# hyeeiin/ECG-Multimodal-Model

Hardware: AMD Instinct MI355X
Metric: samples/sec fwd+bwd, batch-256 multimodal (img+sig+clin), 1->8 MI355X (higher is better)
Workload: dtype bf16; 1 GPU; full multimodal (image 3x224x224 + 5000-pt signal + 16-dim clinical), fwd+bwd+Adam, encoders unfrozen; image_hw=224x224, per_gpu_batch=256, global_batch=256, parallelism=dp1

## Files before the change

ecg-multimodal-model_amd/csrc/conv_stem.hip:

```cpp
#include "ops.h"

__device__ __host__ inline size_t align_up_dev(size_t a) { return (a + 15) & ~(size_t)15; }

#ifndef STEM_ABL
#define STEM_ABL 0
#endif

namespace {

constexpr int STEM_CO = 64;
constexpr int MAXG = 24;

struct StemParams {
  const float* x;
  const void* wpk;
  void* y;
  const float* bias;
  float* stats;
  float* slab;
  int N, Cin, H, W, OH, OW, R, pad_h;
  int TH, TW;
  int tiles_h, tiles_w;
  int NG;
};

template <typename T> struct StemCfg;
template <> struct StemCfg<bf16_t> { static constexpr int WPAD = 8; };
template <> struct StemCfg<float> { static constexpr int WPAD = 4; };

template <int R> struct StemDims {
  static constexpr int TH = R == 1 ? 1 : 8, TW = R == 1 ? 128 : 16;
  static constexpr int PH = (TH - 1) * 2 + R, PW = (TW - 1) * 2 + 8, PWS = (PW + 1) & ~1;
  static constexpr int NPRE = R == 1 ? 16 : 10;
};

template <int R>
__device__ __forceinline__ void stem_patch_offsets(const StemParams& p, int oh0, int ow0,
                                                   unsigned (&off)[StemDims<R>::NPRE]) {
  constexpr int PH = StemDims<R>::PH, PW = StemDims<R>::PW, PWS = StemDims<R>::PWS, NPRE = StemDims<R>::NPRE;
  const int total = p.Cin * PH * PWS;
  const int ih0 = oh0 * 2 - p.pad_h, iw0 = ow0 * 2 - 3;
#pragma unroll
  for (int k = 0; k < NPRE; ++k) {
    const int i = threadIdx.x + 256 * k;
    const int pw = i % PWS;
    const int t = i / PWS;
    const int ph = t % PH, c = t / PH;
    const int ih = ih0 + ph, iw = iw0 + pw;
    const int ok = (int)(i < total) & (int)(pw < PW) & (int)((unsigned)ih < (unsigned)p.H) &
                   (int)((unsigned)iw < (unsigned)p.W);
    off[k] = ok ? (unsigned)((c * p.H + ih) * p.W + iw) * 4u : 0xFFFFFFFFu;
  }
}
template <int R>
__device__ __forceinline__ void stem_fetch_image_patch(const StemParams& p, const unsigned (&off)[StemDims<R>::NPRE],
                                                       float (&pre)[StemDims<R>::NPRE], int n) {
  const size_t img = (size_t)p.Cin * p.H * p.W;
  const __amdgpu_buffer_rsrc_t rs = __builtin_amdgcn_make_buffer_rsrc((void*)(p.x + (size_t)n * img), 0,
                                                                      (int)(img * sizeof(float)), 0x00020000);
#pragma unroll
  for (int k = 0; k < StemDims<R>::NPRE; ++k) {
#if defined(__HIP_DEVICE_COMPILE__)
    pre[k] = __builtin_bit_cast(float, __builtin_amdgcn_raw_buffer_load_b32(rs, (int)off[k], 0, 0));
#endif
  }
}
template <typename T, int R>
__device__ __forceinline__ void stem_store_slots(T* patch, const float (&pre)[StemDims<R>::NPRE]) {
#pragma unroll
  for (int k = 0; k < StemDims<R>::NPRE; ++k) {
    if constexpr (sizeof(T) == 2) patch[threadIdx.x + 256 * k] = f2bf(pre[k]);
    else patch[threadIdx.x + 256 * k] = pre[k];
  }
}

__device__ __forceinline__ int stem_xcd_order() {
  const int nwg = gridDim.x, q = nwg >> 3, r = nwg & 7, xcd = blockIdx.x & 7, k = blockIdx.x >> 3;
  return (xcd < r ? xcd * (q + 1) : r * (q + 1) + (xcd - r) * q) + k;
}

template <typename T, int R, int SMODE = 0>
__global__ __launch_bounds__(256) void stem_fwd_kernel(StemParams p) {
  constexpr bool STATS_ONLY = SMODE == 1, STATS_WG = SMODE != 0;
  extern __shared__ __attribute__((aligned(16))) unsigned char smem[];
  constexpr int TH = StemDims<R>::TH, TW = StemDims<R>::TW, PH = StemDims<R>::PH, PWS = StemDims<R>::PWS;
  constexpr int NPRE = StemDims<R>::NPRE, PB = NPRE * 256;
  constexpr int VEC = Elem<T>::VEC;
  constexpr int KSMAX = (MAXG + 3) / 4;
  const int ksteps = (p.NG + 3) / 4;
  const int KP = ksteps * 32;
  const int WS = KP + StemCfg<T>::WPAD;
  T* sW = reinterpret_cast<T*>(smem);
  T* const patch0 = reinterpret_cast<T*>(smem + align_up_dev((size_t)STEM_CO * WS * sizeof(T)));

  const int tid = threadIdx.x, lane = tid & 63, wave = tid >> 6;
  const int fr = lane & 15, fq = lane >> 4;

  {
    const T* wg = (const T*)p.wpk;
    const int vpr = KP / VEC;
    for (int i = tid; i < STEM_CO * vpr; i += 256) {
      int co = i / vpr, kv = i - co * vpr;
      *reinterpret_cast<u32x4*>(sW + co * WS + kv * VEC) = *reinterpret_cast<const u32x4*>(wg + (size_t)co * KP + kv * VEC);
    }
  }
  const int tpi = p.tiles_h * p.tiles_w;
  const int vb = stem_xcd_order();
  const int pos = vb % tpi, slot = vb / tpi, nslots = gridDim.x / tpi;
  const int th_i = pos / p.tiles_w, tw_i = pos - th_i * p.tiles_w;
  const int oh0 = th_i * TH, ow0 = tw_i * TW;

  float pre[NPRE];
  unsigned poff[NPRE];
  stem_patch_offsets<R>(p, oh0, ow0, poff);

  constexpr int segs = TW / 16;
  int prow[2], pcol[2], boff[2], oofs[2];
  bool okb[2];
#pragma unroll
  for (int b = 0; b < 2; ++b) {
    const int t = wave * 2 + b;
    prow[b] = t / segs;
    pcol[b] = (t % segs) * 16 + fr;
    boff[b] = prow[b] * 2 * PWS + pcol[b] * 2;
    okb[b] = (oh0 + prow[b] < p.OH) & (ow0 + pcol[b] < p.OW);
    oofs[b] = ((oh0 + prow[b]) * p.OW + ow0 + pcol[b]) * STEM_CO;
  }
  unsigned goff2[KSMAX / 2];
#pragma unroll
  for (int ks = 0; ks < KSMAX; ++ks) {
    int G = ks * 4 + fq;
    if (G >= p.NG) G = p.NG - 1;
    const int c = G / R, r = G - c * R;
    const unsigned g = (unsigned)((c * PH + r) * PWS);
    if (ks & 1) goff2[ks / 2] |= g << 16;
    else goff2[ks / 2] = g;
  }
  const T* wlane = sW + fr * WS + fq * 8;

  float ws1[STATS_WG ? 4 : 1][4], ws2[STATS_WG ? 4 : 1][4];
  if (STATS_WG) {
#pragma unroll
    for (int a = 0; a < 4; ++a)
#pragma unroll
      for (int j = 0; j < 4; ++j) ws1[a][j] = ws2[a][j] = 0.f;
  }
  int n = slot;
  if (n < p.N) {
    stem_fetch_image_patch<R>(p, poff, pre, n);
    stem_store_slots<T, R>(patch0, pre);
  }
  __syncthreads();
  for (int cur = 0; n < p.N; n += nslots, cur ^= 1) {
  const T* patch = patch0 + cur * PB;
  const bool has_next = n + nslots < p.N;
  if (has_next && (STEM_ABL != 4 || p.N < 0)) stem_fetch_image_patch<R>(p, poff, pre, n + nslots);

  f32x4 acc[4][2];
  if constexpr (sizeof(T) != 2) {
#pragma unroll
    for (int a = 0; a < 4; ++a)
#pragma unroll
      for (int b = 0; b < 2; ++b) acc[a][b] = (f32x4){0.f, 0.f, 0.f, 0.f};
  }

  if constexpr (sizeof(T) == 2) {
#pragma unroll
    for (int ks = 0; ks < KSMAX; ++ks) {
      if (ks < ksteps && (STEM_ABL != 3 || p.N < 0)) {
        u32x4 fb[2];
#pragma unroll
        for (int b = 0; b < 2; ++b) {
          const int goff = (ks & 1) ? (int)(goff2[ks / 2] >> 16) : (int)(goff2[ks / 2] & 0xffffu);
          const unsigned* src = reinterpret_cast<const unsigned*>(patch + goff + boff[b]);
          fb[b] = (u32x4){src[0], src[1], src[2], src[3]};
        }
#pragma unroll
        for (int a = 0; a < 4; ++a) {
          u32x4 fa = *reinterpret_cast<const u32x4*>(wlane + a * 16 * WS + ks * 32);
#pragma unroll
          for (int b = 0; b < 2; ++b) {
            if (ks == 0) mfma_bf16_first(acc[a][b], fa, fb[b]);
            else mfma_bf16_inplace(acc[a][b], fa, fb[b]);
          }
        }
      }
    }
    mfma_drain();
  } else {
    for (int ks = 0; ks < ksteps; ++ks) {
#pragma unroll
      for (int g = 0; g < 4; ++g) {
        int G2 = ks * 4 + g;
        if (G2 >= p.NG) G2 = p.NG - 1;
        const int c2 = G2 / R, r2 = G2 - c2 * R;
#pragma unroll
        for (int hf = 0; hf < 2; ++hf) {
          const int s = hf * 4 + fq;
          float fbv[2];
#pragma unroll
          for (int b = 0; b < 2; ++b) fbv[b] = patch[(c2 * PH + r2) * PWS + boff[b] + s];
#pragma unroll
          for (int a = 0; a < 4; ++a) {
            float fav = sW[(a * 16 + fr) * WS + (ks * 4 + g) * 8 + s];
#pragma unroll
            for (int b = 0; b < 2; ++b)
              acc[a][b] = __builtin_amdgcn_mfma_f32_16x16x4f32(fav, fbv[b], acc[a][b], 0, 0, 0);
          }
        }
      }
    }
  }

  if (has_next) stem_store_slots<T, R>(patch0 + (cur ^ 1) * PB, pre);
  if constexpr (STATS_ONLY) {
#pragma unroll
    for (int a = 0; a < 4; ++a)
#pragma unroll
      for (int b = 0; b < 2; ++b)
        if (okb[b]) {
#pragma unroll
          for (int j = 0; j < 4; ++j) {
            const float v = p.bias ? acc[a][b][j] + p.bias[a * 16 + fq * 4 + j] : acc[a][b][j];
            ws1[a][j] += v;
            ws2[a][j] += v * v;
          }
        }
    __syncthreads();
    continue;
  }
  T* yimg = (T*)p.y + (size_t)n * p.OH * p.OW * STEM_CO;
  const int tile = n * tpi + pos;
  const __amdgpu_buffer_rsrc_t yrs = __builtin_amdgcn_make_buffer_rsrc(
      (void*)yimg, 0, (int)((size_t)p.OH * p.OW * STEM_CO * sizeof(T)), 0x00020000);
  const __amdgpu_buffer_rsrc_t srs = __builtin_amdgcn_make_buffer_rsrc(
      (void*)(p.stats ? p.stats + (size_t)tile * 4 * 2 * STEM_CO : nullptr), 0, p.stats ? 4 * 2 * STEM_CO * 4 : 0, 0x00020000);
#pragma unroll
  for (int ap = 0; ap < 4; ap += 2) {
  uint2 opk[2][2];
#pragma unroll
  for (int a = ap; a < ap + 2; ++a) {
    const int ch0 = a * 16 + fq * 4;
    float bvv[4] = {0.f, 0.f, 0.f, 0.f};
    if (p.bias) {
#pragma unroll
      for (int j = 0; j < 4; ++j) bvv[j] = p.bias[ch0 + j];
    }
    float s1[4] = {0.f, 0.f, 0.f, 0.f}, s2[4] = {0.f, 0.f, 0.f, 0.f};
#pragma unroll
    for (int b = 0; b < 2; ++b) {
      float v[4];
#pragma unroll
      for (int j = 0; j < 4; ++j) v[j] = p.bias ? acc[a][b][j] + bvv[j] : acc[a][b][j];
      if (okb[b]) {
#pragma unroll
        for (int j = 0; j < 4; ++j) {
          s1[j] += v[j];
          s2[j] += v[j] * v[j];
        }
        if (sizeof(T) != 2) *reinterpret_cast<float4*>(yimg + oofs[b] + ch0) = make_float4(v[0], v[1], v[2], v[3]);
      }
      if (sizeof(T) == 2) {
        opk[a - ap][b].x = (unsigned)f2bf(v[0]) | ((unsigned)f2bf(v[1]) << 16);
        opk[a - ap][b].y = (unsigned)f2bf(v[2]) | ((unsigned)f2bf(v[3]) << 16);
      }
    }
    if (STATS_WG) {
      if (p.stats) {
#pragma unroll
        for (int j = 0; j < 4; ++j) {
          ws1[a][j] += s1[j];
          ws2[a][j] += s2[j];
        }
      }
    } else if (p.stats && (STEM_ABL != 2 || p.N < 0)) {
#pragma unroll
      for (int j = 0; j < 4; ++j) {
        s1[j] = row16_sum(s1[j]);
        s2[j] = row16_sum(s2[j]);
      }
#if defined(__HIP_DEVICE_COMPILE__)
      {
        const unsigned so = fr == 0 ? (unsigned)((wave * 2 * STEM_CO + ch0) * 4) : 0xFFFFFFFFu;
        __builtin_amdgcn_raw_buffer_store_b128((u32x4){__float_as_uint(s1[0]), __float_as_uint(s1[1]), __float_as_uint(s1[2]), __float_as_uint(s1[3])},
                                               srs, (int)so, 0, 0);
        __builtin_amdgcn_raw_buffer_store_b128((u32x4){__float_as_uint(s2[0]), __float_as_uint(s2[1]), __float_as_uint(s2[2]), __float_as_uint(s2[3])},
                                               srs, (int)so, STEM_CO * 4, 0);
      }
#endif
    }
  }
#if defined(__HIP_DEVICE_COMPILE__)
  if (sizeof(T) == 2) {
#pragma unroll
    for (int b = 0; b < 2; ++b) {
      auto lo = __builtin_amdgcn_permlane16_swap(opk[0][b].x, opk[1][b].x, false, false);
      auto hi = __builtin_amdgcn_permlane16_swap(opk[0][b].y, opk[1][b].y, false, false);
      const int ch = (fq & 1) ? (ap + 1) * 16 + (fq - 1) * 4 : ap * 16 + fq * 4;
      const unsigned yo = okb[b] ? (unsigned)(oofs[b] + ch) * 2u : 0xFFFFFFFFu;
      if (STEM_ABL != 1 || p.N < 0)
        __builtin_amdgcn_raw_buffer_store_b128((u32x4){lo[0], hi[0], lo[1], hi[1]}, yrs, (int)yo, 0, 0);
    }
  }
#endif
  }
  __syncthreads();
  }
  if (STATS_WG && p.stats) {
    float* srow = p.stats + ((size_t)blockIdx.x * 4 + wave) * 2 * STEM_CO;
#pragma unroll
    for (int a = 0; a < 4; ++a) {
      f32x4 r1, r2;
#pragma unroll
      for (int j = 0; j < 4; ++j) {
        r1[j] = row16_sum(ws1[a][j]);
        r2[j] = row16_sum(ws2[a][j]);
      }
      if (fr == 0) {
        *reinterpret_cast<f32x4*>(srow + a * 16 + fq * 4) = r1;
        *reinterpret_cast<f32x4*>(srow + STEM_CO + a * 16 + fq * 4) = r2;
      }
    }
  }
}

template <typename T, int R>
__global__ __launch_bounds__(256) void stem_wgrad_kernel(StemParams p) {
  extern __shared__ __attribute__((aligned(16))) unsigned char smem[];
  constexpr int DYS = sizeof(T) == 2 ? 144 : 320;
  constexpr int TH = StemDims<R>::TH, TW = StemDims<R>::TW, PH = StemDims<R>::PH, PWS = StemDims<R>::PWS;
  unsigned char* sDY = smem;
  float* patch = reinterpret_cast<float*>(smem + 128 * DYS);

  const int tid = threadIdx.x, lane = tid & 63, wave = tid >> 6;
  const int fr = lane & 15, fq = lane >> 4;
  const int NK = p.NG * 8;
  const int ktiles = (NK + 15) / 16;
  const int tpi = p.tiles_h * p.tiles_w;
  const int vb = stem_xcd_order();
  const int pos = vb % tpi, slot = vb / tpi, nslots = gridDim.x / tpi;
  const int th_i = pos / p.tiles_w, tw_i = pos - th_i * p.tiles_w;
  const int oh0 = th_i * TH, ow0 = tw_i * TW;

  f32x4 acc[4][3];
#pragma unroll
  for (int a = 0; a < 4; ++a)
#pragma unroll
    for (int b = 0; b < 3; ++b) acc[a][b] = (f32x4){0.f, 0.f, 0.f, 0.f};

  int koff[3];
#pragma unroll
  for (int b = 0; b < 3; ++b) {
    const int kidx = (wave + 4 * b) * 16 + fr;
    const bool kok = (wave + 4 * b) < ktiles && kidx < NK;
    const int kk = kok ? kidx : 0;
    const int G = kk >> 3, c = G / R;
    koff[b] = (c * PH + (G - c * R)) * PWS + (kk & 7);
  }

  const T* dy = (const T*)p.y;
  constexpr int CH = 64 * (int)sizeof(T) / 16;
  constexpr int NDY = 128 * CH / 256;
  float pre[StemDims<R>::NPRE];
  u32x4 pdy[NDY];
  unsigned poff[StemDims<R>::NPRE], dyoff[NDY];
  stem_patch_offsets<R>(p, oh0, ow0, poff);
#pragma unroll
  for (int k = 0; k < NDY; ++k) {
    const int i = tid + 256 * k;
    const int pix = i / CH, chunk = i % CH;
    const int oh = oh0 + pix / TW, ow = ow0 + pix % TW;
    dyoff[k] = ((oh < p.OH) & (ow < p.OW)) ? (unsigned)(((oh * p.OW + ow) * STEM_CO) * (int)sizeof(T) + chunk * 16) : 0xFFFFFFFFu;
  }
  auto fetch = [&](int n) {
    const size_t dimg = (size_t)p.OH * p.OW * STEM_CO;
    const __amdgpu_buffer_rsrc_t drs = __builtin_amdgcn_make_buffer_rsrc((void*)(dy + (size_t)n * dimg), 0,
                                                                          (int)(dimg * sizeof(T)), 0x00020000);
#pragma unroll
    for (int k = 0; k < NDY; ++k) {
#if defined(__HIP_DEVICE_COMPILE__)
      pdy[k] = __builtin_amdgcn_raw_buffer_load_b128(drs, (int)dyoff[k], 0, 0);
#endif
    }
    stem_fetch_image_patch<R>(p, poff, pre, n);
  };
  if (slot < p.N) fetch(slot);
  for (int n = slot; n < p.N; n += nslots) {
    __syncthreads();
#pragma unroll
    for (int k = 0; k < NDY; ++k) {
      const int i = tid + 256 * k;
      *reinterpret_cast<u32x4*>(sDY + (i / CH) * DYS + (i % CH) * 16) = pdy[k];
    }
    stem_store_slots<float, R>(patch, pre);
    __syncthreads();
    if (n + nslots < p.N) fetch(n + nslots);

    if constexpr (sizeof(T) == 2) {
      const int q = fr >> 2, pq = fr & 3;
      for (int st = 0; st < 4; ++st) {
        u32x4 fa[4];
#pragma unroll
        for (int a = 0; a < 4; ++a) {
          const unsigned char* a0 = sDY + (st * 32 + 8 * fq + q) * DYS + (a * 16 + 4 * pq) * 2;
          s16x4 lo = __builtin_amdgcn_ds_read_tr16_b64_v4i16(
              (__attribute__((address_space(3))) s16x4*)(const_cast<unsigned char*>(a0)));
          s16x4 hi = __builtin_amdgcn_ds_read_tr16_b64_v4i16(
              (__attribute__((address_space(3))) s16x4*)(const_cast<unsigned char*>(a0 + 4 * DYS)));
          uint2 l2 = __builtin_bit_cast(uint2, lo), h2 = __builtin_bit_cast(uint2, hi);
          fa[a] = (u32x4){l2.x, l2.y, h2.x, h2.y};
        }
        const int pix0 = st * 32 + 8 * fq;
        const int trow = pix0 / TW, tcol0 = pix0 % TW;
#pragma unroll
        for (int b = 0; b < 3; ++b) {
          float bv[8];
          const float* src = patch + koff[b] + trow * 2 * PWS + tcol0 * 2;
#pragma unroll
          for (int j = 0; j < 8; ++j) bv[j] = src[2 * j];
          u32x4 fb = pack16<bf16_t>(bv);
#pragma unroll
          for (int a = 0; a < 4; ++a)
            mfma_bf16_inplace(acc[a][b], fa[a], fb);
        }
      }
    } else {
      for (int st = 0; st < 32; ++st) {
        const int pix = st * 4 + fq;
        const int trow = pix / TW, tcol = pix % TW;
        float fa[4];
#pragma unroll
        for (int a = 0; a < 4; ++a) fa[a] = *reinterpret_cast<const float*>(sDY + pix * DYS + (a * 16 + fr) * 4);
#pragma unroll
        for (int b = 0; b < 3; ++b) {
          float fb = patch[koff[b] + trow * 2 * PWS + tcol * 2];
#pragma unroll
          for (int a = 0; a < 4; ++a) acc[a][b] = __builtin_amdgcn_mfma_f32_16x16x4f32(fa[a], fb, acc[a][b], 0, 0, 0);
        }
      }
    }
  }

  if (sizeof(T) == 2) mfma_drain();
#pragma unroll
  for (int b = 0; b < 3; ++b) {
    int kidx = (wave + 4 * b) * 16 + fr;
    if ((wave + 4 * b) >= ktiles || kidx >= NK) continue;
#pragma unroll
    for (int a = 0; a < 4; ++a)
#pragma unroll
      for (int j = 0; j < 4; ++j)
        p.slab[((size_t)blockIdx.x * STEM_CO + a * 16 + fq * 4 + j) * NK + kidx] = acc[a][b][j];
  }
}

__global__ __launch_bounds__(256) void stem_wgrad_reduce_kernel(const float* __restrict__ slab,
                                                                float* __restrict__ grad, int nsplit, int NG,
                                                                int accumulate) {
  __shared__ float sh[16][17];
  const int oi = threadIdx.x & 15, sl = threadIdx.x >> 4;
  const int i = blockIdx.x * 16 + oi;
  const int total = STEM_CO * NG * 7;
  const int NK = NG * 8;
  float acc = 0.f;
  if (i < total) {
    int s = i % 7;
    int t = i / 7;
    int G = t % NG, co = t / NG;
    const float* src = slab + (size_t)co * NK + G * 8 + s;
    const size_t stride = (size_t)STEM_CO * NK;
    int k = sl;
    for (; k + 48 < nsplit; k += 64) {
      const float a0 = src[(size_t)k * stride], a1 = src[(size_t)(k + 16) * stride];
      const float a2 = src[(size_t)(k + 32) * stride], a3 = src[(size_t)(k + 48) * stride];
      acc += a0;
      acc += a1;
      acc += a2;
      acc += a3;
    }
    for (; k < nsplit; k += 16) acc += src[(size_t)k * stride];
  }
  sh[sl][oi] = acc;
  __syncthreads();
  if (sl == 0 && i < total) {
    float v = 0.f;
    for (int k = 0; k < 16; ++k) v += sh[k][oi];
    grad[i] = accumulate ? grad[i] + v : v;
  }
}

template <typename T>
__global__ void stem_pack_kernel(const float* __restrict__ w, T* __restrict__ out, int NG, int KP) {
  int i = blockIdx.x * blockDim.x + threadIdx.x;
  if (i >= STEM_CO * KP) return;
  int co = i / KP, k = i - co * KP;
  int G = k >> 3, s = k & 7;
  float v = (G < NG && s < 7) ? w[((size_t)co * NG + G) * 7 + s] : 0.f;
  Elem<T>::st(out + i, v);
}

struct StemShape {
  int OH, OW, TH, TW, tiles_h, tiles_w, NG, KP;
};
int stem_shape(int Cin, int H, int W, int R, StemShape& s) {
  if (R != 1 && R != 7) ECG_FAIL(ECGMM_ERR_SHAPE, "stem: R=%d (1 or 7)", R);
  s.NG = Cin * R;
  if (s.NG > MAXG) ECG_FAIL(ECGMM_ERR_SHAPE, "stem: Cin*R=%d > %d", s.NG, MAXG);
  int pad_h = R / 2;
  s.OH = (H + 2 * pad_h - R) / 2 + 1;
  s.OW = (W + 6 - 7) / 2 + 1;
  if (R == 1) { s.TH = 1; s.TW = 128; }
  else { s.TH = 8; s.TW = 16; }
  s.tiles_h = ceil_div(s.OH, s.TH);
  s.tiles_w = ceil_div(s.OW, s.TW);
  s.KP = ((s.NG + 3) / 4) * 32;
  {
    int PH = (s.TH - 1) * 2 + R, PW = (s.TW - 1) * 2 + 8, PWS = (PW + 1) & ~1;
    if ((double)Cin * H * W * 4.0 >= 2147483648.0 || (double)s.OH * s.OW * STEM_CO * 4.0 >= 2147483648.0)
      ECG_FAIL(ECGMM_ERR_SHAPE, "stem: one sample of %d x %d x %d exceeds the 2 GiB buffer-addressing range", Cin, H, W);
    if (Cin * PH * PWS > (R == 1 ? 16 : 10) * 256) ECG_FAIL(ECGMM_ERR_SHAPE, "stem: input patch of %d channels exceeds the prefetch registers", Cin);
  }
  return 0;
}
void fill_params(StemParams& p, const StemShape& s, int N, int Cin, int H, int W, int R) {
  memset(&p, 0, sizeof(p));
  p.N = N; p.Cin = Cin; p.H = H; p.W = W; p.OH = s.OH; p.OW = s.OW; p.R = R; p.pad_h = R / 2;
  p.TH = s.TH; p.TW = s.TW; p.tiles_h = s.tiles_h; p.tiles_w = s.tiles_w; p.NG = s.NG;
}
size_t stem_patch_buffer_bytes(int R, size_t esz) { return (size_t)(R == 1 ? 16 : 10) * 256 * esz; }
size_t patch_bytes(const StemShape& s, int Cin, int R) {
  int PH = (s.TH - 1) * 2 + R, PW = (s.TW - 1) * 2 + 8, PWS = (PW + 1) & ~1;
  return (size_t)Cin * PH * PWS * sizeof(float);
}

}

size_t ecg_stem_packed_elems(int Cin, int R) { return (size_t)STEM_CO * (((Cin * R + 3) / 4) * 32); }
int ecg_stem_stats_rows(int N, int Cin, int H, int W, int R) {
  StemShape s;
  if (stem_shape(Cin, H, W, R, s)) return -1;
  return 4 * N * s.tiles_h * s.tiles_w;
}

int ecg_stem_pack(int dtype, const float* w, void* out, int Cin, int R, hipStream_t stream) {
  int NG = Cin * R, KP = ((NG + 3) / 4) * 32;
  int n = STEM_CO * KP;
  if (dtype == ECGMM_BF16)
    hipLaunchKernelGGL(stem_pack_kernel<bf16_t>, dim3(ceil_div(n, 256)), dim3(256), 0, stream, w, (bf16_t*)out, NG, KP);
  else
    hipLaunchKernelGGL(stem_pack_kernel<float>, dim3(ceil_div(n, 256)), dim3(256), 0, stream, w, (float*)out, NG, KP);
  ECG_CHECK_LAUNCH("stem_pack");
  return 0;
}

int ecg_stem_wg_stats_rows(int N, int Cin, int H, int W, int R) { return ecg_stem_stats_only_rows(N, Cin, H, W, R); }
static int stem_fwd_impl(int dtype, const float* x, const void* wpk, const float* bias, void* y, float* stats, int N, int Cin,
                         int H, int W, int R, bool wg_rows, hipStream_t stream);
int ecg_stem_fwd_wgrows(int dtype, const float* x, const void* wpk, const float* bias, void* y, float* stats, int N, int Cin,
                        int H, int W, int R, hipStream_t stream) {
  return stem_fwd_impl(dtype, x, wpk, bias, y, stats, N, Cin, H, W, R, true, stream);
}
int ecg_stem_fwd(int dtype, const float* x, const void* wpk, const float* bias, void* y, float* stats, int N, int Cin,
                 int H, int W, int R, hipStream_t stream) {
  return stem_fwd_impl(dtype, x, wpk, bias, y, stats, N, Cin, H, W, R, false, stream);
}
static int stem_fwd_impl(int dtype, const float* x, const void* wpk, const float* bias, void* y, float* stats, int N, int Cin,
                         int H, int W, int R, bool wg_rows, hipStream_t stream) {
  StemShape s;
  ECG_TRY(stem_shape(Cin, H, W, R, s));
  StemParams p;
  fill_params(p, s, N, Cin, H, W, R);
  p.x = x; p.wpk = wpk; p.y = y; p.bias = bias; p.stats = stats;
  const size_t esz = dtype_size(dtype);
  const int WS = s.KP + (dtype == ECGMM_BF16 ? 8 : 4);
  size_t lds = align_up((size_t)STEM_CO * WS * esz, 16) + 2 * stem_patch_buffer_bytes(R, esz);
  const int tpi = s.tiles_h * s.tiles_w;
  int nslots = 2048 / tpi;
  nslots = nslots < 1 ? 1 : (nslots > N ? N : nslots);
  dim3 grid(tpi * nslots);
  ecg_prof_begin(ECG_PROF_STEM_FWD, 2.0 * (double)N * s.OH * s.OW * STEM_CO * Cin * R * 7,
                 4.0 * N * Cin * H * W + (double)dtype_size(dtype) * N * s.OH * s.OW * STEM_CO, stream);
  if (dtype == ECGMM_BF16 && wg_rows) {
    if (R == 7) hipLaunchKernelGGL((stem_fwd_kernel<bf16_t, 7, 2>), grid, dim3(256), lds, stream, p);
    else hipLaunchKernelGGL((stem_fwd_kernel<bf16_t, 1, 2>), grid, dim3(256), lds, stream, p);
  } else if (wg_rows) {
    ECG_FAIL(ECGMM_ERR_DTYPE, "stem: per-workgroup statistics rows are a bf16 form");
  } else if (dtype == ECGMM_BF16) {
    if (R == 7) hipLaunchKernelGGL((stem_fwd_kernel<bf16_t, 7>), grid, dim3(256), lds, stream, p);
    else hipLaunchKernelGGL((stem_fwd_kernel<bf16_t, 1>), grid, dim3(256), lds, stream, p);
  } else if (dtype == ECGMM_F32) {
    static bool once = false;
    if (!once) {
      (void)hipFuncSetAttribute((const void*)stem_fwd_kernel<float, 7>, hipFuncAttributeMaxDynamicSharedMemorySize, 100 * 1024);
      (void)hipFuncSetAttribute((const void*)stem_fwd_kernel<float, 1>, hipFuncAttributeMaxDynamicSharedMemorySize, 100 * 1024);
      once = true;
    }
    if (R == 7) hipLaunchKernelGGL((stem_fwd_kernel<float, 7>), grid, dim3(256), lds, stream, p);
    else hipLaunchKernelGGL((stem_fwd_kernel<float, 1>), grid, dim3(256), lds, stream, p);
  } else {
    ECG_FAIL(ECGMM_ERR_DTYPE, "stem: bad dtype %d", dtype);
  }
  ecg_prof_end(stream);
  ECG_CHECK_LAUNCH("stem_fwd");
  return 0;
}

static int stem_stats_grid(int N, int tpi) {
  int nslots = 2048 / tpi;
  nslots = nslots < 1 ? 1 : (nslots > N ? N : nslots);
  return tpi * nslots;
}
int ecg_stem_stats_only_rows(int N, int Cin, int H, int W, int R) {
  StemShape s;
  if (stem_shape(Cin, H, W, R, s)) return -1;
  return 4 * stem_stats_grid(N, s.tiles_h * s.tiles_w);
}
int ecg_stem_stats_only(int dtype, const float* x, const void* wpk, const float* bias, float* stats, int N, int Cin,
                        int H, int W, int R, hipStream_t stream) {
  if (dtype != ECGMM_BF16) ECG_FAIL(ECGMM_ERR_DTYPE, "stem statistics-only pass: bf16 only");
  StemShape s;
  ECG_TRY(stem_shape(Cin, H, W, R, s));
  StemParams p;
  fill_params(p, s, N, Cin, H, W, R);
  p.x = x; p.wpk = wpk; p.bias = bias; p.stats = stats;
  const int WS = s.KP + 8;
  size_t lds = align_up((size_t)STEM_CO * WS * 2, 16) + 2 * stem_patch_buffer_bytes(R, 2);
  dim3 grid(stem_stats_grid(N, s.tiles_h * s.tiles_w));
  ecg_prof_begin(ECG_PROF_STEM_FWD, 2.0 * (double)N * s.OH * s.OW * STEM_CO * Cin * R * 7, 4.0 * N * Cin * H * W, stream);
  if (R == 7) hipLaunchKernelGGL((stem_fwd_kernel<bf16_t, 7, 1>), grid, dim3(256), lds, stream, p);
  else hipLaunchKernelGGL((stem_fwd_kernel<bf16_t, 1, 1>), grid, dim3(256), lds, stream, p);
  ecg_prof_end(stream);
  ECG_CHECK_LAUNCH("stem_stats_only");
  return 0;
}

int ecg_stem_wgrad_reduce(const float* slab, float* grad, int rows, int NG, int accumulate, hipStream_t stream) {
  hipLaunchKernelGGL(stem_wgrad_reduce_kernel, dim3(ceil_div(STEM_CO * NG * 7, 16)), dim3(256), 0, stream, slab, grad, rows, NG,
                     accumulate);
  ECG_CHECK_LAUNCH("stem_wgrad_reduce");
  return 0;
}

static int stem_wgrad_grid(int N, int tpi) {
  int nslots = 1024 / tpi;
  nslots = nslots < 1 ? 1 : (nslots > N ? N : nslots);
  return tpi * nslots;
}

size_t ecg_stem_wgrad_workspace(int N, int Cin, int H, int W, int R) {
  StemShape s;
  if (stem_shape(Cin, H, W, R, s)) return 0;
  return (size_t)stem_wgrad_grid(N, s.tiles_h * s.tiles_w) * STEM_CO * s.NG * 8 * sizeof(float);
}

int ecg_stem_wgrad(int dtype, const float* x, const void* dy, float* grad, int accumulate, void* workspace,
                   size_t workspace_bytes, int N, int Cin, int H, int W, int R, hipStream_t stream) {
  StemShape s;
  ECG_TRY(stem_shape(Cin, H, W, R, s));
  const int grid = stem_wgrad_grid(N, s.tiles_h * s.tiles_w);
  size_t need = (size_t)grid * STEM_CO * s.NG * 8 * sizeof(float);
  if (!workspace || workspace_bytes < need)
    ECG_FAIL(ECGMM_ERR_WORKSPACE, "stem wgrad: workspace %zu < %zu", workspace_bytes, need);
  StemParams p;
  fill_params(p, s, N, Cin, H, W, R);
  p.x = x; p.y = const_cast<void*>(dy); p.slab = (float*)workspace;
  size_t lds = 128 * (size_t)(dtype == ECGMM_BF16 ? 144 : 320) + stem_patch_buffer_bytes(R, sizeof(float));
  if (dtype != ECGMM_BF16 && dtype != ECGMM_F32) ECG_FAIL(ECGMM_ERR_DTYPE, "stem wgrad: bad dtype %d", dtype);
  ecg_prof_begin(ECG_PROF_STEM_WGRAD, 2.0 * (double)N * s.OH * s.OW * STEM_CO * Cin * R * 7,
                 4.0 * N * Cin * H * W + (double)dtype_size(dtype) * N * s.OH * s.OW * STEM_CO, stream);
  if (dtype == ECGMM_BF16) {
    if (R == 7) hipLaunchKernelGGL((stem_wgrad_kernel<bf16_t, 7>), dim3(grid), dim3(256), lds, stream, p);
    else hipLaunchKernelGGL((stem_wgrad_kernel<bf16_t, 1>), dim3(grid), dim3(256), lds, stream, p);
  } else {
    if (R == 7) hipLaunchKernelGGL((stem_wgrad_kernel<float, 7>), dim3(grid), dim3(256), lds, stream, p);
    else hipLaunchKernelGGL((stem_wgrad_kernel<float, 1>), dim3(grid), dim3(256), lds, stream, p);
  }
  ecg_prof_end(stream);
  ECG_CHECK_LAUNCH("stem_wgrad");
  hipLaunchKernelGGL(stem_wgrad_reduce_kernel, dim3(ceil_div(STEM_CO * s.NG * 7, 16)), dim3(256), 0, stream,
                     (const float*)workspace, grad, grid, s.NG, accumulate);
  ECG_CHECK_LAUNCH("stem_wgrad_reduce");
  return 0;
}
```

Baseline: 39150 samples/s.

## Specialize stem conv k-steps, cache bias in LDS, parity-split bf16 wgrad patch

```diff
diff --git a/ecg-multimodal-model_amd/csrc/conv_stem.hip b/ecg-multimodal-model_amd/csrc/conv_stem.hip
--- a/ecg-multimodal-model_amd/csrc/conv_stem.hip
+++ b/ecg-multimodal-model_amd/csrc/conv_stem.hip
@@ -32,6 +32,7 @@
   static constexpr int TH = R == 1 ? 1 : 8, TW = R == 1 ? 128 : 16;
   static constexpr int PH = (TH - 1) * 2 + R, PW = (TW - 1) * 2 + 8, PWS = (PW + 1) & ~1;
   static constexpr int NPRE = R == 1 ? 16 : 10;
+  static constexpr int PWH = (PW / 2 + 7) & ~7;
 };
 
 template <int R>
@@ -74,20 +75,41 @@
   }
 }
 
+template <int R>
+__device__ __forceinline__ void stem_parity_slots(const StemParams& p, unsigned (&dst2)[StemDims<R>::NPRE / 2]) {
+  constexpr int PH = StemDims<R>::PH, PWS = StemDims<R>::PWS, PWH = StemDims<R>::PWH, NPRE = StemDims<R>::NPRE;
+  const int total = p.Cin * PH * PWS;
+#pragma unroll
+  for (int k = 0; k < NPRE; ++k) {
+    const int i = threadIdx.x + 256 * k;
+    const int pw = i % PWS, row = i / PWS;
+    const unsigned d = i < total ? (unsigned)((row * 2 + (pw & 1)) * PWH + (pw >> 1)) : (unsigned)(PWH - 1);
+    if (k & 1) dst2[k / 2] |= d << 16;
+    else dst2[k / 2] = d;
+  }
+}
+template <int R>
+__device__ __forceinline__ void stem_store_parity(bf16_t* patch, const float (&pre)[StemDims<R>::NPRE],
+                                                  const unsigned (&dst2)[StemDims<R>::NPRE / 2]) {
+#pragma unroll
+  for (int k = 0; k < StemDims<R>::NPRE; ++k)
+    patch[(k & 1) ? dst2[k / 2] >> 16 : dst2[k / 2] & 0xffffu] = f2bf(pre[k]);
+}
+
 __device__ __forceinline__ int stem_xcd_order() {
   const int nwg = gridDim.x, q = nwg >> 3, r = nwg & 7, xcd = blockIdx.x & 7, k = blockIdx.x >> 3;
   return (xcd < r ? xcd * (q + 1) : r * (q + 1) + (xcd - r) * q) + k;
 }
 
-template <typename T, int R, int SMODE = 0>
+template <typename T, int R, int SMODE = 0, int KS = 0>
 __global__ __launch_bounds__(256) void stem_fwd_kernel(StemParams p) {
   constexpr bool STATS_ONLY = SMODE == 1, STATS_WG = SMODE != 0;
   extern __shared__ __attribute__((aligned(16))) unsigned char smem[];
   constexpr int TH = StemDims<R>::TH, TW = StemDims<R>::TW, PH = StemDims<R>::PH, PWS = StemDims<R>::PWS;
   constexpr int NPRE = StemDims<R>::NPRE, PB = NPRE * 256;
   constexpr int VEC = Elem<T>::VEC;
-  constexpr int KSMAX = (MAXG + 3) / 4;
-  const int ksteps = (p.NG + 3) / 4;
+  constexpr int KSMAX = KS ? KS : (MAXG + 3) / 4;
+  const int ksteps = KS ? KS : (p.NG + 3) / 4;
   const int KP = ksteps * 32;
   const int WS = KP + StemCfg<T>::WPAD;
   T* sW = reinterpret_cast<T*>(smem);
@@ -104,6 +126,8 @@
       *reinterpret_cast<u32x4*>(sW + co * WS + kv * VEC) = *reinterpret_cast<const u32x4*>(wg + (size_t)co * KP + kv * VEC);
     }
   }
+  float* const sBias = reinterpret_cast<float*>(patch0 + 2 * PB);
+  if (p.bias && tid < STEM_CO) sBias[tid] = p.bias[tid];
   const int tpi = p.tiles_h * p.tiles_w;
   const int vb = stem_xcd_order();
   const int pos = vb % tpi, slot = vb / tpi, nslots = gridDim.x / tpi;
@@ -126,7 +150,7 @@
     okb[b] = (oh0 + prow[b] < p.OH) & (ow0 + pcol[b] < p.OW);
     oofs[b] = ((oh0 + prow[b]) * p.OW + ow0 + pcol[b]) * STEM_CO;
   }
-  unsigned goff2[KSMAX / 2];
+  unsigned goff2[(KSMAX + 1) / 2];
 #pragma unroll
   for (int ks = 0; ks < KSMAX; ++ks) {
     int G = ks * 4 + fq;
@@ -164,7 +188,34 @@
       for (int b = 0; b < 2; ++b) acc[a][b] = (f32x4){0.f, 0.f, 0.f, 0.f};
   }
 
-  if constexpr (sizeof(T) == 2) {
+  if constexpr (sizeof(T) == 2 && KS > 0) {
+    if (STEM_ABL != 3 || p.N < 0) {
+      u32x4 fa[2][4], fb[2][2];
+      auto read_step = [&](int ks, u32x4 (&a4)[4], u32x4 (&b2)[2]) {
+        const int goff = (ks & 1) ? (int)(goff2[ks / 2] >> 16) : (int)(goff2[ks / 2] & 0xffffu);
+#pragma unroll
+        for (int b = 0; b < 2; ++b) {
+          const unsigned* src = reinterpret_cast<const unsigned*>(patch + goff + boff[b]);
+          b2[b] = (u32x4){src[0], src[1], src[2], src[3]};
+        }
+#pragma unroll
+        for (int a = 0; a < 4; ++a) a4[a] = *reinterpret_cast<const u32x4*>(wlane + a * 16 * WS + ks * 32);
+      };
+      read_step(0, fa[0], fb[0]);
+#pragma unroll
+      for (int ks = 0; ks < KS; ++ks) {
+        if (ks + 1 < KS) read_step(ks + 1, fa[(ks + 1) & 1], fb[(ks + 1) & 1]);
+#pragma unroll
+        for (int a = 0; a < 4; ++a)
+#pragma unroll
+          for (int b = 0; b < 2; ++b) {
+            if (ks == 0) mfma_bf16_first(acc[a][b], fa[0][a], fb[0][b]);
+            else mfma_bf16_inplace(acc[a][b], fa[ks & 1][a], fb[ks & 1][b]);
+          }
+      }
+    }
+    mfma_drain();
+  } else if constexpr (sizeof(T) == 2) {
 #pragma unroll
     for (int ks = 0; ks < KSMAX; ++ks) {
       if (ks < ksteps && (STEM_ABL != 3 || p.N < 0)) {
@@ -221,7 +272,7 @@
         if (okb[b]) {
 #pragma unroll
           for (int j = 0; j < 4; ++j) {
-            const float v = p.bias ? acc[a][b][j] + p.bias[a * 16 + fq * 4 + j] : acc[a][b][j];
+            const float v = p.bias ? acc[a][b][j] + sBias[a * 16 + fq * 4 + j] : acc[a][b][j];
             ws1[a][j] += v;
             ws2[a][j] += v * v;
           }
@@ -244,7 +295,7 @@
     float bvv[4] = {0.f, 0.f, 0.f, 0.f};
     if (p.bias) {
 #pragma unroll
-      for (int j = 0; j < 4; ++j) bvv[j] = p.bias[ch0 + j];
+      for (int j = 0; j < 4; ++j) bvv[j] = sBias[ch0 + j];
     }
     float s1[4] = {0.f, 0.f, 0.f, 0.f}, s2[4] = {0.f, 0.f, 0.f, 0.f};
 #pragma unroll
@@ -329,8 +380,10 @@
   extern __shared__ __attribute__((aligned(16))) unsigned char smem[];
   constexpr int DYS = sizeof(T) == 2 ? 144 : 320;
   constexpr int TH = StemDims<R>::TH, TW = StemDims<R>::TW, PH = StemDims<R>::PH, PWS = StemDims<R>::PWS;
+  constexpr int PWH = StemDims<R>::PWH;
+  constexpr bool PAR = sizeof(T) == 2;
   unsigned char* sDY = smem;
-  float* patch = reinterpret_cast<float*>(smem + 128 * DYS);
+  T* patch = reinterpret_cast<T*>(smem + 128 * DYS);
 
   const int tid = threadIdx.x, lane = tid & 63, wave = tid >> 6;
   const int fr = lane & 15, fq = lane >> 4;
@@ -355,8 +408,10 @@
     const bool kok = (wave + 4 * b) < ktiles && kidx < NK;
     const int kk = kok ? kidx : 0;
     const int G = kk >> 3, c = G / R;
-    koff[b] = (c * PH + (G - c * R)) * PWS + (kk & 7);
-  }
+    koff[b] = PAR ? ((c * PH + (G - c * R)) * 2 + (kk & 1)) * PWH : (c * PH + (G - c * R)) * PWS + (kk & 7);
+  }
+  const bool sh_dword = (fr & 4) != 0;
+  const unsigned sh_bits = (fr & 2) ? 16u : 0u;
 
   const T* dy = (const T*)p.y;
   constexpr int CH = 64 * (int)sizeof(T) / 16;
@@ -365,6 +420,8 @@
   u32x4 pdy[NDY];
   unsigned poff[StemDims<R>::NPRE], dyoff[NDY];
   stem_patch_offsets<R>(p, oh0, ow0, poff);
+  unsigned pdst2[StemDims<R>::NPRE / 2];
+  if constexpr (PAR) stem_parity_slots<R>(p, pdst2);
 #pragma unroll
   for (int k = 0; k < NDY; ++k) {
     const int i = tid + 256 * k;
@@ -392,14 +449,20 @@
       const int i = tid + 256 * k;
       *reinterpret_cast<u32x4*>(sDY + (i / CH) * DYS + (i % CH) * 16) = pdy[k];
     }
-    stem_store_slots<float, R>(patch, pre);
+    if constexpr (PAR) stem_store_parity<R>(patch, pre, pdst2);
+    else stem_store_slots<float, R>(patch, pre);
     __syncthreads();
     if (n + nslots < p.N) fetch(n + nslots);
 
     if constexpr (sizeof(T) == 2) {
       const int q = fr >> 2, pq = fr & 3;
-      for (int st = 0; st < 4; ++st) {
-        u32x4 fa[4];
+      struct BRaw { u32x4 lo; uint2 hi; };
+      u32x4 fa[4];
+      BRaw fbr[3];
+      const bf16_t* bsrc[3];
+#pragma unroll
+      for (int b = 0; b < 3; ++b) bsrc[b] = patch + koff[b] + (8 * fq / TW) * 4 * PWH + (8 * fq) % TW;
+      auto read_step = [&](int st, u32x4 (&a4)[4], BRaw (&b3)[3]) {
 #pragma unroll
         for (int a = 0; a < 4; ++a) {
           const unsigned char* a0 = sDY + (st * 32 + 8 * fq + q) * DYS + (a * 16 + 4 * pq) * 2;
@@ -408,20 +471,32 @@
           s16x4 hi = __builtin_amdgcn_ds_read_tr16_b64_v4i16(
               (__attribute__((address_space(3))) s16x4*)(const_cast<unsigned char*>(a0 + 4 * DYS)));
           uint2 l2 = __builtin_bit_cast(uint2, lo), h2 = __builtin_bit_cast(uint2, hi);
-          fa[a] = (u32x4){l2.x, l2.y, h2.x, h2.y};
-        }
-        const int pix0 = st * 32 + 8 * fq;
-        const int trow = pix0 / TW, tcol0 = pix0 % TW;
+          a4[a] = (u32x4){l2.x, l2.y, h2.x, h2.y};
+        }
+        static_assert(TW == 16 || TW == 128, "a 32-pixel step is two whole tile rows or a quarter of one");
+        constexpr int STEP = TW == 16 ? 2 * 4 * PWH : 32;
 #pragma unroll
         for (int b = 0; b < 3; ++b) {
-          float bv[8];
-          const float* src = patch + koff[b] + trow * 2 * PWS + tcol0 * 2;
-#pragma unroll
-          for (int j = 0; j < 8; ++j) bv[j] = src[2 * j];
-          u32x4 fb = pack16<bf16_t>(bv);
-#pragma unroll
-          for (int a = 0; a < 4; ++a)
-            mfma_bf16_inplace(acc[a][b], fa[a], fb);
+          const bf16_t* src = bsrc[b] + st * STEP;
+          b3[b].lo = *reinterpret_cast<const u32x4*>(src);
+          b3[b].hi = *reinterpret_cast<const uint2*>(src + 8);
+        }
+      };
+      auto b_frag = [&](const BRaw& r) {
+        auto pick = [&](unsigned d0, unsigned d1) { return sh_dword ? d1 : d0; };
+        const unsigned e0 = pick(r.lo[0], r.lo[1]), e1 = pick(r.lo[1], r.lo[2]), e2 = pick(r.lo[2], r.lo[3]);
+        const unsigned e3 = pick(r.lo[3], r.hi.x), e4 = pick(r.hi.x, r.hi.y);
+        return (u32x4){__builtin_amdgcn_alignbit(e1, e0, sh_bits), __builtin_amdgcn_alignbit(e2, e1, sh_bits),
+                       __builtin_amdgcn_alignbit(e3, e2, sh_bits), __builtin_amdgcn_alignbit(e4, e3, sh_bits)};
+      };
+#pragma unroll
+      for (int st = 0; st < 4; ++st) {
+        read_step(st, fa, fbr);
+#pragma unroll
+        for (int b = 0; b < 3; ++b) {
+          const u32x4 fb = b_frag(fbr[b]);
+#pragma unroll
+          for (int a = 0; a < 4; ++a) mfma_bf16_inplace(acc[a][b], fa[a], fb);
         }
       }
     } else {
@@ -528,6 +603,18 @@
   p.TH = s.TH; p.TW = s.TW; p.tiles_h = s.tiles_h; p.tiles_w = s.tiles_w; p.NG = s.NG;
 }
 size_t stem_patch_buffer_bytes(int R, size_t esz) { return (size_t)(R == 1 ? 16 : 10) * 256 * esz; }
+
+template <int SMODE>
+void stem_fwd_launch_bf16(const StemParams& p, dim3 grid, size_t lds, hipStream_t stream) {
+  if (p.R == 7) {
+    if (p.Cin == 3) hipLaunchKernelGGL((stem_fwd_kernel<bf16_t, 7, SMODE, 6>), grid, dim3(256), lds, stream, p);
+    else hipLaunchKernelGGL((stem_fwd_kernel<bf16_t, 7, SMODE>), grid, dim3(256), lds, stream, p);
+  } else {
+    if (p.Cin == 1) hipLaunchKernelGGL((stem_fwd_kernel<bf16_t, 1, SMODE, 1>), grid, dim3(256), lds, stream, p);
+    else if (p.Cin == 12) hipLaunchKernelGGL((stem_fwd_kernel<bf16_t, 1, SMODE, 3>), grid, dim3(256), lds, stream, p);
+    else hipLaunchKernelGGL((stem_fwd_kernel<bf16_t, 1, SMODE>), grid, dim3(256), lds, stream, p);
+  }
+}
 size_t patch_bytes(const StemShape& s, int Cin, int R) {
   int PH = (s.TH - 1) * 2 + R, PW = (s.TW - 1) * 2 + 8, PWS = (PW + 1) & ~1;
   return (size_t)Cin * PH * PWS * sizeof(float);
@@ -573,7 +660,8 @@
   p.x = x; p.wpk = wpk; p.y = y; p.bias = bias; p.stats = stats;
   const size_t esz = dtype_size(dtype);
   const int WS = s.KP + (dtype == ECGMM_BF16 ? 8 : 4);
-  size_t lds = align_up((size_t)STEM_CO * WS * esz, 16) + 2 * stem_patch_buffer_bytes(R, esz);
+  size_t lds = align_up((size_t)STEM_CO * WS * esz, 16) + 2 * stem_patch_buffer_bytes(R, esz) +
+               STEM_CO * sizeof(float);
   const int tpi = s.tiles_h * s.tiles_w;
   int nslots = 2048 / tpi;
   nslots = nslots < 1 ? 1 : (nslots > N ? N : nslots);
@@ -581,13 +669,11 @@
   ecg_prof_begin(ECG_PROF_STEM_FWD, 2.0 * (double)N * s.OH * s.OW * STEM_CO * Cin * R * 7,
                  4.0 * N * Cin * H * W + (double)dtype_size(dtype) * N * s.OH * s.OW * STEM_CO, stream);
   if (dtype == ECGMM_BF16 && wg_rows) {
-    if (R == 7) hipLaunchKernelGGL((stem_fwd_kernel<bf16_t, 7, 2>), grid, dim3(256), lds, stream, p);
-    else hipLaunchKernelGGL((stem_fwd_kernel<bf16_t, 1, 2>), grid, dim3(256), lds, stream, p);
+    stem_fwd_launch_bf16<2>(p, grid, lds, stream);
   } else if (wg_rows) {
     ECG_FAIL(ECGMM_ERR_DTYPE, "stem: per-workgroup statistics rows are a bf16 form");
   } else if (dtype == ECGMM_BF16) {
-    if (R == 7) hipLaunchKernelGGL((stem_fwd_kernel<bf16_t, 7>), grid, dim3(256), lds, stream, p);
-    else hipLaunchKernelGGL((stem_fwd_kernel<bf16_t, 1>), grid, dim3(256), lds, stream, p);
+    stem_fwd_launch_bf16<0>(p, grid, lds, stream);
   } else if (dtype == ECGMM_F32) {
     static bool once = false;
     if (!once) {
@@ -624,11 +710,10 @@
   fill_params(p, s, N, Cin, H, W, R);
   p.x = x; p.wpk = wpk; p.bias = bias; p.stats = stats;
   const int WS = s.KP + 8;
-  size_t lds = align_up((size_t)STEM_CO * WS * 2, 16) + 2 * stem_patch_buffer_bytes(R, 2);
+  size_t lds = align_up((size_t)STEM_CO * WS * 2, 16) + 2 * stem_patch_buffer_bytes(R, 2) + STEM_CO * sizeof(float);
   dim3 grid(stem_stats_grid(N, s.tiles_h * s.tiles_w));
   ecg_prof_begin(ECG_PROF_STEM_FWD, 2.0 * (double)N * s.OH * s.OW * STEM_CO * Cin * R * 7, 4.0 * N * Cin * H * W, stream);
-  if (R == 7) hipLaunchKernelGGL((stem_fwd_kernel<bf16_t, 7, 1>), grid, dim3(256), lds, stream, p);
-  else hipLaunchKernelGGL((stem_fwd_kernel<bf16_t, 1, 1>), grid, dim3(256), lds, stream, p);
+  stem_fwd_launch_bf16<1>(p, grid, lds, stream);
   ecg_prof_end(stream);
   ECG_CHECK_LAUNCH("stem_stats_only");
   return 0;
@@ -664,7 +749,9 @@
   StemParams p;
   fill_params(p, s, N, Cin, H, W, R);
   p.x = x; p.y = const_cast<void*>(dy); p.slab = (float*)workspace;
-  size_t lds = 128 * (size_t)(dtype == ECGMM_BF16 ? 144 : 320) + stem_patch_buffer_bytes(R, sizeof(float));
+  const int PH = R == 7 ? StemDims<7>::PH : StemDims<1>::PH, PWH = R == 7 ? StemDims<7>::PWH : StemDims<1>::PWH;
+  size_t lds = dtype == ECGMM_BF16 ? 128 * (size_t)144 + (size_t)Cin * PH * 2 * PWH * sizeof(bf16_t)
+                                   : 128 * (size_t)320 + stem_patch_buffer_bytes(R, sizeof(float));
   if (dtype != ECGMM_BF16 && dtype != ECGMM_F32) ECG_FAIL(ECGMM_ERR_DTYPE, "stem wgrad: bad dtype %d", dtype);
   ecg_prof_begin(ECG_PROF_STEM_WGRAD, 2.0 * (double)N * s.OH * s.OW * STEM_CO * Cin * R * 7,
                  4.0 * N * Cin * H * W + (double)dtype_size(dtype) * N * s.OH * s.OW * STEM_CO, stream);
```

After: 39290 samples/s (median of 6 runs). No clear change (+0.4%).
